# MystenLabs/dapol

Hardware: AMD Instinct MI355X
Metric: entities/sec (tree build + 64-bit range-proof gen), 2^20 leaves, 1/2/4/8 GPU (higher is better)
Workload: dtype int32 limbs (255-bit modular integers)

## Files before the change

### dapol_amd/csrc/host_range.inc

```

#include <cstdlib>
#include "policy_plan.inc"
#include "prove_plan.inc"

struct MsmTiming {
    std::vector<hipEvent_t> ev;
    std::vector<int> kind;
    size_t used = 0;
    bool enabled = false;
    size_t kernels[2] = {0, 0};
    ~MsmTiming() { for (auto e : ev) (void)hipEventDestroy(e); }
    hipError_t mark(hipStream_t st, int k = 0) {
        if (!enabled) return hipSuccess;
        if (used == ev.size()) {
            hipEvent_t e;
            hipError_t r = hipEventCreate(&e);
            if (r != hipSuccess) return r;
            ev.push_back(e);
        }
        if ((used & 1) == 0) { if (kind.size() <= used / 2) kind.push_back(k); else kind[used / 2] = k; }
        return hipEventRecord(ev[used++], st);
    }
    void count(int k, size_t n) { if (enabled) kernels[k] += n; }
    double total_ms(int k) {
// ... 159 lines not shown
        if (tm) tm->count(0, 1);
    }
}

static int32_t launch_materialise(dapol_ctx* ctx, const ProvePlan& P, const ProveLane& L, const RangeArgs& A, hipStream_t st, MsmTiming* tm) {
    const size_t cb = A.B, T = (size_t)P.tail_n;
    const unsigned g_tail = (unsigned)(cb * (size_t)(P.tail_n / 32));
    if (P.gs_mat) {
        const int LW = P.mat_LW(), cpl = P.mat_cpl(cb);
        const unsigned g_cls = nblk(cb * (size_t)LW, 64);
        const size_t slot_words = (size_t)4 * FE_NL * cb * LW;
        for (int side = 0; side < 2; side++)
            for (int c0 = 0; c0 < P.tail_n; c0 += MAT_GROUP) {
                const int nc = P.tail_n - c0 < MAT_GROUP ? P.tail_n - c0 : MAT_GROUP;
                for (int c = 0; c < nc; c += cpl) {
                    const int ny = nc - c < cpl ? nc - c : cpl;
                    hipLaunchKernelGGL(k_rp_mat_gs, dim3(g_cls, ny), dim3(64), 0, st, A, ctx->tv, side, c0 + c, 0, LW, L.gsacc + c * slot_words);
                    if (LW < A.nwin) hipLaunchKernelGGL(k_rp_mat_gs, dim3(g_cls, ny), dim3(64), 0, st, A, ctx->tv, side, c0 + c, 1, LW, L.gsacc + c * slot_words);
                }
                hipLaunchKernelGGL(k_rp_mat_gs_horner, dim3(nblk(cb * (size_t)nc, 64)), dim3(64), 0, st, A, side, c0, nc, LW, L.gsacc);
            }
        if (tm) tm->count(1, 2 * (size_t)((P.tail_n + cpl - 1) / cpl) * (LW < A.nwin ? 2 : 1));
    } else if (P.mat_split > 1) {
        RangeArgs Am = A;
        Am.nsplit = P.mat_split; Am.P0 = L.split[2];
        hipLaunchKernelGGL((k_rp_msm<MSM_MATERIALIZE, 32>), dim3(g_tail * (unsigned)P.mat_split), dim3(64), 0, st, Am, ctx->tv, -1); LAUNCH_CHECK();
        hipLaunchKernelGGL(k_rp_sum_mat, dim3(nblk(cb * 2 * T, 64)), dim3(64), 0, st, cb * 2 * T, P.mat_split, Am.P0, A.tailT);
    } else {
        hipLaunchKernelGGL((k_rp_msm<MSM_MATERIALIZE, 32>), dim3(g_tail), dim3(64), 0, st, A, ctx->tv, -1);
        if (tm) tm->count(1, 1);
    }
    LAUNCH_CHECK();
    return DAPOL_OK;
}

static int32_t queue_chunk(dapol_ctx* ctx, const ProvePlan& P, const ProveLane& L, RangeArgs A, hipStream_t st, ForkGuard& fg, uint32_t* d_err,
                           MsmTiming* tm) {
    const size_t cb = A.B;
    const int fs_shape = P.fs_shape, nf_rounds = P.nf_rounds();
    sc* const stab_buf = A.stab;
    if (!P.stab_main) A.stab = nullptr;
    const unsigned g_wave = (unsigned)cb, g_lane = nblk(cb, 64), g_dig = (unsigned)(cb * (size_t)(A.TP / 64));
    const unsigned g_gsdig = nblk(cb * (size_t)(2 * A.N), 64);
    hipLaunchKernelGGL(k_rp_nonce_key, dim3(g_lane), dim3(64), 0, st, A); LAUNCH_CHECK();
    if (P.gs) hipLaunchKernelGGL(k_rp_nonces_gs, dim3(g_gsdig), dim3(64), 0, st, A);
    else hipLaunchKernelGGL(k_rp_nonces, dim3(g_dig), dim3(64), 0, st, A);
    LAUNCH_CHECK();
    if (P.side_A) {
        HIPCHK(hipEventRecord(ctx->ev_fork, st));
        HIPCHK(hipStreamWaitEvent(ctx->side[2], ctx->ev_fork, 0));
        fg.forked(2);
        hipLaunchKernelGGL(k_rp_A, dim3(g_wave), dim3(64), 0, ctx->side[2], A, ctx->tv); LAUNCH_CHECK();
        HIPCHK(hipEventRecord(ctx->ev_join[2], ctx->side[2]));
        FAULT_AFTER_FORK("prove_A");
    } else if (P.a_lane(cb)) {
        hipLaunchKernelGGL(k_rp_A_lane, dim3(g_lane), dim3(64), 0, st, A, ctx->tv); LAUNCH_CHECK();
    } else {
        hipLaunchKernelGGL(k_rp_A, dim3(g_wave), dim3(64), 0, st, A, ctx->tv); LAUNCH_CHECK();
    }
    if (tm) HIPCHK(tm->mark(st));
    launch_main_msm(ctx, P, L, A, st, -1, tm); LAUNCH_CHECK();
    if (tm) HIPCHK(tm->mark(st));
    if (P.side_A) { HIPCHK(hipStreamWaitEvent(st, ctx->ev_join[2], 0)); fg.joined(2); }
    LAUNCH_FS(k_rp_finish1, fs_shape, cb, st, A, ctx->tv); LAUNCH_CHECK();
    hipLaunchKernelGGL(k_rp_poly, dim3(g_wave * (unsigned)A.fs_parts), dim3(64), 0, st, A); LAUNCH_CHECK();
    LAUNCH_FS(k_rp_finish2, fs_shape, cb, st, A, ctx->tv); LAUNCH_CHECK();
    hipLaunchKernelGGL(k_rp_lr, dim3(g_wave * (unsigned)A.fs_parts), dim3(64), 0, st, A); LAUNCH_CHECK();
    if (fs_shape == 2) hipLaunchKernelGGL(k_rp_finish3<2>, dim3(g_wave), dim3(64), 0, st, A);
    else hipLaunchKernelGGL(k_rp_finish3<0>, dim3(g_lane), dim3(64), 0, st, A);
    LAUNCH_CHECK();
    for (int k = 0; k < nf_rounds; k++) {
        if (P.gs) hipLaunchKernelGGL(k_rp_round_prep_gs, dim3(g_gsdig), dim3(64), 0, st, A, k);
        else hipLaunchKernelGGL(k_rp_round_prep, dim3(g_dig), dim3(64), 0, st, A, k);
        LAUNCH_CHECK();
        hipLaunchKernelGGL(k_rp_round_ip, dim3(g_wave), dim3(64), 0, st, A, k); LAUNCH_CHECK();
        if (tm) HIPCHK(tm->mark(st));
        launch_main_msm(ctx, P, L, A, st, k, tm); LAUNCH_CHECK();
        if (tm) HIPCHK(tm->mark(st));
        LAUNCH_FS(k_rp_round_finish, fs_shape, cb, st, A, ctx->tv, k); LAUNCH_CHECK();
        hipLaunchKernelGGL(k_rp_fold, dim3(fold_blocks(A, cb, k)), dim3(256), 0, st, A, k);
        LAUNCH_CHECK();
    }
    if (nf_rounds == A.lgN) {
        hipLaunchKernelGGL(k_rp_final, dim3(g_lane), dim3(64), 0, st, A, d_err); LAUNCH_CHECK();
        return DAPOL_OK;
    }
    if (P.gs_mat) hipLaunchKernelGGL(k_rp_mat_prep_gs, dim3(g_gsdig), dim3(64), 0, st, A);
    else hipLaunchKernelGGL(k_rp_mat_prep, dim3(g_dig), dim3(64), 0, st, A);
    LAUNCH_CHECK();
    if (tm) HIPCHK(tm->mark(st, 1));
    { int32_t rc = launch_materialise(ctx, P, L, A, st, tm); if (rc) return rc; }
    if (tm) HIPCHK(tm->mark(st, 1));
    const unsigned g_tail = (unsigned)(cb * (size_t)(P.tail_n / 32));
    {
        RangeArgs Ai = A;
        Ai.stab = P.stab_tail ? stab_buf : nullptr;
        if (P.tail_rpl == 4) hipLaunchKernelGGL(k_rp_tail_table4, dim3(nblk(cb * (size_t)(2 * P.tail_n / 4), 64)), dim3(64), 0, st, Ai);
        else hipLaunchKernelGGL(k_rp_tail_table, dim3(g_tail), dim3(64), 0, st, Ai);
        LAUNCH_CHECK();
    }
    RangeArgs At = A;
    At.N = P.tail_n; At.lgN = P.tail_lgn; At.TP = 2 * P.tail_n; At.wbits = TAIL_WBITS; At.nwin = TAIL_NWIN; At.nsplit = 0;
    At.a = A.tail_a; At.b = A.tail_b; At.s1 = A.tail_s1; At.s2 = A.tail_s2;
    At.stab = P.stab_tail ? stab_buf : nullptr;
    At.out_round0 = nf_rounds;
    const TableView tvt{A.tailT, 1, TAIL_WBITS, 0, 0};
    for (int k = 0; k < P.tail_lgn; k++) {
        hipLaunchKernelGGL(k_rp_round_prep, dim3(g_tail), dim3(64), 0, st, At, k); LAUNCH_CHECK();
        hipLaunchKernelGGL(k_rp_round_ip, dim3(g_wave), dim3(64), 0, st, At, k); LAUNCH_CHECK();
        if (P.tail_gs) {
            hipLaunchKernelGGL(k_rp_tail_gs, dim3(nblk(2 * cb, TAIL_GS_LISTS)), dim3(TAIL_GS_BLOCK), 0, st, At, tvt, k, L.gsacc); LAUNCH_CHECK();
            hipLaunchKernelGGL(k_rp_tail_combine, dim3(nblk(2 * cb, 64)), dim3(64), 0, st, At, L.gsacc);
        } else launch_msm_tail(st, At, tvt, k, P.tail_lpl);
        LAUNCH_CHECK();
        LAUNCH_FS(k_rp_round_finish, fs_shape, cb, st, At, ctx->tv, k); LAUNCH_CHECK();
        hipLaunchKernelGGL(k_rp_fold, dim3(fold_blocks(At, cb, k)), dim3(256), 0, st, At, k);
        LAUNCH_CHECK();
    }
    hipLaunchKernelGGL(k_rp_final, dim3(g_lane), dim3(64), 0, st, At, d_err); LAUNCH_CHECK();
    return DAPOL_OK;
}

static int32_t range_prove_device(dapol_ctx* ctx, int n, int m, size_t B, const uint64_t* d_vals, const uint32_t* d_blind,
                                  const uint32_t* d_Vc, const uint32_t* d_seed, const uint64_t* d_stream, uint64_t slot_base,
                                  const uint32_t* d_tape, uint32_t* d_out, MsmTiming* tm, size_t tape_stride = 0, uint32_t sub_k = 1,
                                  size_t out_stride = 0, PendingProve* pend = nullptr) {
    ProveShape s{};
    s.n = n; s.m = m; s.B = B;
    s.tail_length = ctx->opt.tail_length; s.small_call_max = ctx->opt.small_call_max; s.generator_stationary = ctx->opt.generator_stationary;
    s.streams = ctx->opt.streams; s.gs_tile_rows = ctx->opt.gs_tile_rows; s.gs_slices = ctx->opt.gs_slices; s.chunk_proofs = ctx->opt.chunk_proofs;
    s.wbits = ctx->tv.wbits; s.nwin = ctx->tv.nwin_c(); s.hi_split = ctx->tv.hi_split;
    s.n_cu = ctx->n_cu; s.resident_waves = ctx->resident_waves();
    s.budget_bytes = scratch_budget_bytes(ctx);
    s.timed = tm != nullptr;
    ProvePlan P = plan_range_prove(s);
    for (bool lowered = false;; lowered = true) {
        hipError_t e = ctx->scratch.ensure(P.lane_bytes() * P.nlanes);
        if (e == hipSuccess) {
            if (lowered) P.finalise(s, P.chunk, P.nlanes);
            break;
        }
        (void)hipGetLastError();
        if (e != hipErrorOutOfMemory || (P.nlanes == 1 && P.chunk <= 64)) return fail_hip(e, "scratch allocation", __FILE__, __LINE__);
        if (P.nlanes > 1) P.nlanes--;
        else P.chunk = (P.chunk + 1) / 2;
    }
    const size_t chunk = P.chunk, slots = (size_t)m * (2 * (size_t)n + 4);
    const int nlanes = P.nlanes;
    RangeArgs A{};
    A.n = n; A.m = m; A.N = P.N; A.lgN = P.lgN; A.TP = P.TP;
    A.out_words = 72 + 16 * A.lgN;
    A.seed = d_seed; A.slot_base = slot_base;
    A.wbits = s.wbits; A.nwin = s.nwin;
    A.tail_n = P.tail_n; A.use_hi = P.use_hi ? 1 : 0; A.fs_parts = P.fs_parts; A.mat_round = P.nf_rounds();
    A.stream_id = d_stream;
    A.tape_stride = (uint32_t)(tape_stride ? tape_stride : slots);
    A.tape = d_tape;
    A.sub_k = sub_k ? sub_k : 1; A.sub_slots = (uint32_t)slots;
    A.out = d_out; A.out_stride = out_stride ? out_stride : (size_t)A.out_words;
    ProveLane lanes[4];
    hipStream_t lane_stream[4] = {ctx->stream, ctx->side[0], ctx->side[1], ctx->side[2]};
    for (int ln = 0; ln < nlanes; ln++) lanes[ln] = carve_lane(P, A, (uint8_t*)ctx->scratch.p + P.lane_bytes() * ln);
    DevBuf<uint32_t> err_own;
    DevBuf<uint32_t>& err = pend ? pend->err : err_own;
    HIPCHK(err.alloc(1));
    HIPCHK(hipMemsetAsync(err.p, 0, 4, ctx->stream));
    ForkGuard fg(ctx);
    if (nlanes > 1) {
        HIPCHK(hipEventRecord(ctx->ev_fork, ctx->stream));
        for (int ln = 1; ln < nlanes; ln++) { HIPCHK(hipStreamWaitEvent(lane_stream[ln], ctx->ev_fork, 0)); fg.forked(ln - 1); }
    }
    size_t chunk_no = 0;
    for (size_t first = 0; first < B; first += chunk, chunk_no++) {
        const int ln = (int)(chunk_no % (size_t)nlanes);
        if (chunk_no == 2) FAULT_AFTER_FORK("prove_lanes");
        RangeArgs Ac = lanes[ln].A;
        Ac.B = B - first < chunk ? B - first : chunk;
        Ac.vals = d_vals + first * m;
        Ac.blind = d_blind + first * m * 8;
        Ac.Vc = d_Vc + first * m * 8;
        Ac.p0 = first;
        int32_t rc = queue_chunk(ctx, P, lanes[ln], Ac, lane_stream[ln], fg, err.p, tm);
        if (rc) return rc;
    }
    for (int ln = 1; ln < nlanes; ln++) {
        HIPCHK(hipEventRecord(ctx->ev_join[ln - 1], lane_stream[ln]));
        HIPCHK(hipStreamWaitEvent(ctx->stream, ctx->ev_join[ln - 1], 0));
        fg.joined(ln - 1);
    }
    if (pend) {
        pend->ctx = ctx;
        pend->h_err_p = ctx->h_pinned + pend->pinned_slot;
        HIPCHK(hipMemcpyAsync(pend->h_err_p, err.p, 4, hipMemcpyDeviceToHost, ctx->stream));
        pend->armed = true;
        return DAPOL_OK;
    }
    uint32_t h_err = 0;
    HIPCHK(hipMemcpyAsync(&h_err, err.p, 4, hipMemcpyDeviceToHost, ctx->stream));
    HIPCHK(hipStreamSynchronize(ctx->stream));
    if (h_err) return fail(DAPOL_ERR_INVALID_ARGUMENT, "prover drew a zero challenge (ProofError::MaliciousDealer)");
    return DAPOL_OK;
}

struct EventPair {
    hipEvent_t a = nullptr, b = nullptr;
    ~EventPair() { if (a) (void)hipEventDestroy(a); if (b) (void)hipEventDestroy(b); }
    hipError_t init() { hipError_t e = hipEventCreate(&a); return e != hipSuccess ? e : hipEventCreate(&b); }
};

int32_t dapol_range_prove_batch(dapol_ctx* ctx, int32_t n_bits, int32_t m, size_t b, const uint64_t* v, const uint8_t* r32,
                                const uint8_t nonce_seed32[32], const uint64_t* stream_id, uint64_t slot_base, const uint8_t* tape,
                                uint8_t* proofs_out) {
    if (!ctx || (b && (!v || !r32 || !proofs_out))) return fail(DAPOL_ERR_INVALID_ARGUMENT, "null argument");
    if (!tape && (!nonce_seed32 || (b && !stream_id))) return fail(DAPOL_ERR_INVALID_ARGUMENT, "seed mode needs nonce_seed32 and stream_id");
    size_t ps = dapol_range_proof_size(n_bits, m);
    if (ps == 0) return fail(DAPOL_ERR_INVALID_ARGUMENT, "n_bits must be 8/16/32/64 and m a power of two");
    if (m > ctx->max_parties) return fail(DAPOL_ERR_INVALID_ARGUMENT, "m exceeds the context's max_parties (InvalidGeneratorsLength)");
    if (b == 0) return DAPOL_OK;
    HIPCHK(hipSetDevice(ctx->device));
    hipStream_t st = ctx->stream;
    const size_t tot = b * (size_t)m, slots = (size_t)m * (2 * (size_t)n_bits + 4);
    DevBuf<uint64_t> dv, dstream;
    DevBuf<uint32_t> dr, dVc, dseed, dtape, dout;
    HIPCHK(dv.alloc(tot)); HIPCHK(dr.alloc(tot * 8)); HIPCHK(dVc.alloc(tot * 8)); HIPCHK(dseed.alloc(8));
    HIPCHK(dout.alloc(b * ps / 4));
    HIPCHK(hipMemcpyAsync(dv.p, v, tot * 8, hipMemcpyHostToDevice, st));
    HIPCHK(hipMemcpyAsync(dr.p, r32, tot * 32, hipMemcpyHostToDevice, st));
    if (tape) {
        HIPCHK(dtape.alloc(b * slots * 16));
        HIPCHK(hipMemcpyAsync(dtape.p, tape, b * slots * 64, hipMemcpyHostToDevice, st));
        HIPCHK(hipMemsetAsync(dseed.p, 0, 32, st));
    } else {
        HIPCHK(dstream.alloc(b));
        HIPCHK(hipMemcpyAsync(dstream.p, stream_id, b * 8, hipMemcpyHostToDevice, st));
        HIPCHK(hipMemcpyAsync(dseed.p, nonce_seed32, 32, hipMemcpyHostToDevice, st));
    }
    hipLaunchKernelGGL(k_rp_commit_V, dim3(nblk(tot, 256)), dim3(256), 0, st, ctx->tv, tot, dv.p, dr.p, dVc.p);
    LAUNCH_CHECK();
    EventPair ev;
    HIPCHK(ev.init());
    HIPCHK(hipEventRecord(ev.a, st));
    int32_t rc = range_prove_device(ctx, n_bits, m, b, dv.p, dr.p, dVc.p, dseed.p, dstream.p, slot_base, dtape.p, dout.p, nullptr);
    if (rc) return rc;
    HIPCHK(hipEventRecord(ev.b, st));
    HIPCHK(hipMemcpy(proofs_out, dout.p, b * ps, hipMemcpyDeviceToHost));
    { float ms = 0; if (hipEventElapsedTime(&ms, ev.a, ev.b) == hipSuccess) g_last_range_prove_ms.store((double)ms, std::memory_order_relaxed); }
    return DAPOL_OK;
}
```

### dapol_amd/csrc/kernels_range.h

```cpp
#pragma once
#include <hip/hip_runtime.h>
#include <type_traits>
#include "kernels_ctx_tree.h"
#include "ge_quad.h"

namespace dapol {

struct ProofState {
    uint64_t strobe[25];
    uint32_t pos, pos_begin;
    uint32_t err, pad_;
    sc y, z, y_inv, x, w, u, u_inv;
    sc a_bl, s_bl, t1, t2, t1_bl, t2_bl, t_x, cL, cR;
    uint32_t nkey[8];
};

struct RangeArgs {
    int n, m, N, lgN, TP;
    int wbits, nwin;
    size_t B;
    const uint64_t* vals;
    const uint32_t* blind;
    const uint32_t* Vc;
    const uint32_t* seed;
    const uint64_t* stream_id;
    uint64_t slot_base;
    const uint32_t* tape;
    uint32_t tape_stride;
    uint32_t sub_k, sub_slots;
    size_t p0;
    sc* a; sc* b; sc* s1; sc* s2;
    sc* stab;
    dig_t* dig;
    int nsplit;
    int use_hi;
    int fs_parts;
    sc* fs_part;
    ProofState* st;
    int32_t* PA; int32_t* P0; int32_t* P1;
    int mat_round;
    int tail_n;
    int32_t* tailT;
    sc* tail_a; sc* tail_b; sc* tail_s1; sc* tail_s2;
    uint32_t* out;
    size_t out_stride;
    int out_words;
    int out_round0;
};

#ifndef DAPOL_TAIL_WBITS
#define DAPOL_TAIL_WBITS 5
#endif
enum { TAIL_WBITS = DAPOL_TAIL_WBITS, TAIL_NWIN = 253 / TAIL_WBITS + 1, TAIL_ENTRIES = (1 << (TAIL_WBITS - 1)) + 1, TAIL_ROW_WORDS = TAIL_ENTRIES * 32 };
enum { MSM_PLAIN = 0, MSM_MATERIALIZE = 1, MSM_TAIL = 2 };
enum { STAB_ROUNDS = 6, STAB_N = 1 << STAB_ROUNDS };

__device__ __forceinline__ void proof_row(const RangeArgs& A, size_t b, size_t& e, uint32_t& j) {
    const size_t g = A.p0 + b;
    if (A.sub_k <= 1) { e = g; j = 0; }
    else { e = g / A.sub_k; j = (uint32_t)(g - e * A.sub_k); }
}
__device__ __forceinline__ uint32_t* proof_out(const RangeArgs& A, size_t b) {
    size_t e; uint32_t j;
    proof_row(A, b, e, j);
    return A.out + e * A.out_stride + (size_t)j * (size_t)A.out_words;
}
__device__ __forceinline__ void tape_wide(uint32_t* w16, const RangeArgs& A, size_t b, uint32_t slot) {
    size_t e; uint32_t j;
    proof_row(A, b, e, j);
    const uint32_t first = j * A.sub_slots;
    if (A.tape) {
        const uint4* p = reinterpret_cast<const uint4*>(A.tape + (e * (size_t)A.tape_stride + first + slot) * 16);
        for (int i = 0; i < 4; i++) { uint4 q = p[i]; w16[4 * i] = q.x; w16[4 * i + 1] = q.y; w16[4 * i + 2] = q.z; w16[4 * i + 3] = q.w; }
    } else {
        uint32_t key[8];
        for (int i = 0; i < 8; i++) key[i] = A.st[b].nkey[i];
        seed_wide(w16, key, 2u, A.stream_id[e], A.slot_base + first + slot);
    }
}
__global__ __launch_bounds__(64) void k_rp_nonce_key(RangeArgs A) {
    size_t b = (size_t)blockIdx.x * 64 + threadIdx.x;
    if (b >= A.B || A.tape) return;
    uint32_t key[8], w[16];
    for (int i = 0; i < 8; i++) key[i] = A.seed[i];
    size_t e; uint32_t sj;
    proof_row(A, b, e, sj);
    seed_wide(w, key, 6u, A.stream_id[e], A.slot_base + (uint64_t)sj * A.sub_slots);
    for (int i = 0; i < 8; i++) key[i] = w[i];
    seed_wide(w, key, 7u, (uint64_t)A.n, (uint64_t)A.m);
    for (int i = 0; i < 8; i++) key[i] = w[i];
    for (int j0 = 0; j0 < A.m; j0 += 31) {
        const int n_ent = 1 + ((A.m - j0 < 31) ? A.m - j0 : 31);
        const int n_blk = (n_ent + 1) / 2;
        uint32_t cv[8], blk[16], o[16];
        blake3_iv(cv);
        for (int i = 0; i < n_blk; i++) {
            for (int h = 0; h < 2; h++) {
                const int e = 2 * i + h;
                if (e == 0) { for (int k = 0; k < 8; k++) blk[k] = key[k]; }
                else if (e < n_ent) ld8(blk + 8 * h, A.Vc + (b * A.m + j0 + e - 1) * 8);
                else { for (int k = 0; k < 8; k++) blk[8 + k] = 0; }
            }
            const bool last = i == n_blk - 1;
            blake3_compress(o, cv, blk, 0, (last && (n_ent & 1)) ? 32u : 64u, (i == 0 ? B3_CHUNK_START : 0u) | (last ? (B3_CHUNK_END | B3_ROOT) : 0u));
            for (int k = 0; k < 8; k++) cv[k] = o[k];
        }
        for (int k = 0; k < 8; k++) key[k] = cv[k];
    }
    for (int i = 0; i < 8; i++) A.st[b].nkey[i] = key[i];
}
__device__ __forceinline__ void tape_scalar(sc& r, const RangeArgs& A, size_t b, uint32_t slot) {
    uint32_t w[16];
    tape_wide(w, A, b, slot);
    sc_from_wide(r, w);
}
__device__ __forceinline__ void ld_sc(sc& r, const sc* p) {
    const uint4* q = reinterpret_cast<const uint4*>(p);
    uint4 a = q[0], b = q[1];
    r.v[0] = a.x; r.v[1] = a.y; r.v[2] = a.z; r.v[3] = a.w; r.v[4] = b.x; r.v[5] = b.y; r.v[6] = b.z; r.v[7] = b.w;
}
__device__ __forceinline__ void st_sc(sc* p, const sc& r) {
    uint4* q = reinterpret_cast<uint4*>(p);
    q[0] = make_uint4(r.v[0], r.v[1], r.v[2], r.v[3]);
    q[1] = make_uint4(r.v[4], r.v[5], r.v[6], r.v[7]);
}
__device__ __forceinline__ void write_digits_plain(const RangeArgs& A, size_t b, int pos, const uint32_t* c) {
    dig_t* d = A.dig + (size_t)b * A.nwin * A.TP + pos;
    const int TP = A.TP;
    sc_recode_w(A.wbits, A.nwin, c, [&](int i, int digit) { d[(size_t)i * TP] = (dig_t)digit; });
}
__device__ __forceinline__ void write_digits(const RangeArgs& A, size_t b, int pos, const sc& s_mont) {
    uint32_t c[8];
    sc_from_mont(c, s_mont);
    write_digits_plain(A, b, pos, c);
}
__device__ __forceinline__ void zero_digits(const RangeArgs& A, size_t b, int pos) {
    dig_t* d = A.dig + (size_t)b * A.nwin * A.TP + pos;
    for (int i = 0; i < A.nwin; i++) d[(size_t)i * A.TP] = 0;
}

__device__ __forceinline__ void coeff_times(sc& p, const RangeArgs& A, size_t b, int round, int j, bool isH, const sc& v) {
    if (A.stab) {
        const sc* T = A.stab + ((b * 2 + (size_t)(round & 1)) * 2 + (isH ? 1 : 0)) * STAB_N + (round ? (j >> (A.lgN - round)) : 0);
        sc t;
        ld_sc(t, T);
        if (isH) {
            sc yi, q;
            ld_sc(yi, A.s2 + b * A.N + j);
            sc_montmul(q, v, yi);
            sc_montmul(p, q, t);
        } else sc_montmul(p, v, t);
    } else {
        sc sv;
        ld_sc(sv, (isH ? A.s2 : A.s1) + b * A.N + j);
        sc_montmul(p, v, sv);
    }
}
__device__ __forceinline__ void coeff_plain(sc& s, const RangeArgs& A, size_t b, int round, int j, bool isH) {
    if (A.stab) {
        const sc* T = A.stab + ((b * 2 + (size_t)(round & 1)) * 2 + (isH ? 1 : 0)) * STAB_N + (round ? (j >> (A.lgN - round)) : 0);
        sc t;
        ld_sc(t, T);
        if (isH) {
            sc yi;
            ld_sc(yi, A.s2 + b * A.N + j);
            sc_montmul(s, yi, t);
        } else s = t;
    } else ld_sc(s, (isH ? A.s2 : A.s1) + b * A.N + j);
}
__device__ __forceinline__ void stab_init(const RangeArgs& A, size_t b) {
    if (!A.stab) return;
    sc one_p, one_m;
    sc_zero(one_p); one_p.v[0] = 1;
    sc_one_mont(one_m);
    st_sc(A.stab + (b * 2 * 2 + 0) * STAB_N, one_p);
    st_sc(A.stab + (b * 2 * 2 + 1) * STAB_N, one_m);
}

__device__ __forceinline__ int term_generator(int round, int N, int lgN, int side, int q, bool& isH) {
    if (round < 0) {
        isH = side != 0;
        return q;
    }
    int lgh = lgN - 1 - round;
    int half = 1 << lgh, Nh = N >> 1;
    isH = q >= Nh;
// ... 944 lines not shown
```

### dapol_amd/csrc/kernels_range_gs.h

```cpp
#pragma once
#include "kernels_range.h"

namespace dapol {

__device__ __forceinline__ void write_digits_gs(const RangeArgs& A, size_t p, int sp, const uint32_t* c) {
    const size_t L = A.B * (size_t)A.nwin;
    int32_t* out = reinterpret_cast<int32_t*>(A.dig) + ((((size_t)(sp >> 2)) * L + p) << 2) + (sp & 3);
    const size_t wstride = A.B * (size_t)4;
    const int W = A.wbits, NW = A.nwin, half = 1 << (W - 1);
    const uint32_t mask = (1u << W) - 1;
    uint32_t x[8];
#pragma unroll
    for (int i = 0; i < 8; i++) x[i] = c[i];
    int carry = 0;
#pragma nounroll
    for (int w = 0; w < NW; w++) {
        const int b = (int)(x[0] & mask) + carry;
        carry = (b >= half && w != NW - 1) ? 1 : 0;
        out[(size_t)w * wstride] = b - (carry << W);
#pragma unroll
        for (int i = 0; i < 7; i++) x[i] = (x[i] >> W) | (x[i + 1] << (32 - W));
        x[7] >>= W;
    }
}

#define GS_BLOCKS(A, vb) for (size_t vb = blockIdx.x, nb_ = ((size_t)(A).B * (size_t)(2 * (A).N) + 63) / 64; vb < nb_; vb += gridDim.x)
__device__ __forceinline__ bool gs_thread(const RangeArgs& A, size_t vblock, size_t& p, int& sp) {
    const size_t t = vblock * 64 + threadIdx.x;
    const size_t quad = t >> 2, sp4 = quad / A.B;
    p = quad - sp4 * A.B;
    sp = (int)(4 * sp4) + (int)(t & 3);
    return sp4 < (size_t)(2 * A.N) / 4;
}

__global__ __launch_bounds__(64) void k_rp_nonces_gs(RangeArgs A) {
    GS_BLOCKS(A, vb) {
        size_t p;
        int sp;
        if (!gs_thread(A, vb, p, sp)) continue;
        const int side = sp >= A.N ? 1 : 0, q = sp - side * A.N;
        const int j = q / A.n, ii = q - j * A.n;
        const uint32_t slot = (uint32_t)(j * (2 * A.n + 2) + 2 + ii + (side ? A.n : 0));
        sc s;
        tape_scalar(s, A, p, slot);
        st_sc((side ? A.s2 : A.s1) + p * A.N + q, s);
        uint32_t c[8];
        sc_from_mont(c, s);
        write_digits_gs(A, p, sp, c);
    }
}

__global__ __launch_bounds__(64) void k_rp_round_prep_gs(RangeArgs A, int round) {
    GS_BLOCKS(A, vb) {
        size_t p;
        int sp;
        if (!gs_thread(A, vb, p, sp)) continue;
        const int side = sp >= A.N ? 1 : 0, q = sp - side * A.N;
        const int lgh = A.lgN - 1 - round, half = 1 << lgh;
        bool isH;
        const int j = term_generator(round, A.N, A.lgN, side, q, isH);
        const int off = j & (half - 1);
        const bool upper = (j >> lgh) & 1;
        const int vi = upper ? off : off + half;
        sc v, pr;
        ld_sc(v, (isH ? A.b : A.a) + p * A.N + vi);
        coeff_times(pr, A, p, round, j, isH, v);
        write_digits_gs(A, p, sp, pr.v);
    }
}

#ifndef DAPOL_GS_OCC
#define DAPOL_GS_OCC 4
#endif
__global__ __launch_bounds__(64, DAPOL_GS_OCC) void k_rp_msm_gs(RangeArgs A, TableView tbl, int round, int side, int q0, int nq, int first, int32_t* __restrict__ accs, int slice_rows) {
    const size_t L = A.B * (size_t)A.nwin, Ltot = L * gridDim.y;
    const size_t lane = (size_t)blockIdx.x * 64 + threadIdx.x;
    if (lane >= L) return;
    q0 += (int)blockIdx.y * slice_rows;
    ge_p3 acc;
    int32_t* ap = accs + (size_t)blockIdx.y * L + lane;
    if (first) ge_identity(acc);
    else {
#pragma unroll
        for (int i = 0; i < FE_NL; i++) {
            acc.X.v[i] = ap[(size_t)i * Ltot]; acc.Y.v[i] = ap[(size_t)(FE_NL + i) * Ltot];
            acc.Z.v[i] = ap[(size_t)(2 * FE_NL + i) * Ltot]; acc.T.v[i] = ap[(size_t)(3 * FE_NL + i) * Ltot];
        }
    }
    const dapol_v4i* dg = reinterpret_cast<const dapol_v4i*>(A.dig) + ((size_t)(side * A.N + q0) >> 2) * L + lane;
    dapol_v4i d4 = dg[0], dn = d4;
#pragma nounroll
    for (int i = 0; i < nq; i++) {
        if ((i & 3) == 0 && i + 4 < nq) dn = dg[(size_t)((i >> 2) + 1) * L];
        const int d = d4.x;
        d4.x = d4.y; d4.y = d4.z; d4.z = d4.w;
        if ((i & 3) == 3) d4 = dn;
        bool isH;
        const int j = term_generator(round, A.N, A.lgN, side, q0 + i, isH);
        tbl_madd(acc, tbl, gen_row(tbl, A.n, j, isH), d);
    }
#pragma unroll
    for (int i = 0; i < FE_NL; i++) {
        ap[(size_t)i * Ltot] = acc.X.v[i]; ap[(size_t)(FE_NL + i) * Ltot] = acc.Y.v[i];
        ap[(size_t)(2 * FE_NL + i) * Ltot] = acc.Z.v[i]; ap[(size_t)(3 * FE_NL + i) * Ltot] = acc.T.v[i];
    }
}

__global__ __launch_bounds__(64, DAPOL_GS_OCC) void k_rp_msm_gs_hi(RangeArgs A, TableView tbl, int round, int side, int q0, int nq, int first, int32_t* __restrict__ accs,
                                                                  int slice_rows, int LW) {
    const size_t L = A.B * (size_t)LW, Ltot = L * gridDim.y, Ld = A.B * (size_t)A.nwin;
    const size_t lane = (size_t)blockIdx.x * 64 + threadIdx.x;
    if (lane >= L) return;
    q0 += (int)blockIdx.y * slice_rows;
    const int w = (int)(lane / A.B);
    const bool has_hi = w + LW < A.nwin;
    ge_p3 acc;
    int32_t* ap = accs + (size_t)blockIdx.y * L + lane;
    if (first) ge_identity(acc);
    else {
#pragma unroll
        for (int i = 0; i < FE_NL; i++) {
            acc.X.v[i] = ap[(size_t)i * Ltot]; acc.Y.v[i] = ap[(size_t)(FE_NL + i) * Ltot];
            acc.Z.v[i] = ap[(size_t)(2 * FE_NL + i) * Ltot]; acc.T.v[i] = ap[(size_t)(3 * FE_NL + i) * Ltot];
        }
    }
    const dapol_v4i* dg = reinterpret_cast<const dapol_v4i*>(A.dig) + ((size_t)(side * A.N + q0) >> 2) * Ld + lane;
    const dapol_v4i* dh = dg + (has_hi ? (size_t)LW * A.B : 0);
    dapol_v4i d4 = dg[0], h4 = dh[0], dn = d4, hn = h4;
#pragma nounroll
    for (int i2 = 0; i2 < 2 * nq; i2++) {
        const int i = i2 >> 1, hi = i2 & 1;
        if (!hi && (i & 3) == 0 && i + 4 < nq) { dn = dg[(size_t)((i >> 2) + 1) * Ld]; hn = dh[(size_t)((i >> 2) + 1) * Ld]; }
        int d;
        if (!hi) { d = d4.x; d4.x = d4.y; d4.y = d4.z; d4.z = d4.w; }
        else {
            d = h4.x;
            h4.x = h4.y; h4.y = h4.z; h4.z = h4.w;
            if ((i & 3) == 3) { d4 = dn; h4 = hn; }
            if (!has_hi) continue;
        }
        bool isH;
        const int j = term_generator(round, A.N, A.lgN, side, q0 + i, isH);
        const int row = gen_row(tbl, A.n, j, isH);
        tbl_madd(acc, tbl, hi ? tbl.row_hi(row) : row, d);
    }
#pragma unroll
    for (int i = 0; i < FE_NL; i++) {
        ap[(size_t)i * Ltot] = acc.X.v[i]; ap[(size_t)(FE_NL + i) * Ltot] = acc.Y.v[i];
        ap[(size_t)(2 * FE_NL + i) * Ltot] = acc.Z.v[i]; ap[(size_t)(3 * FE_NL + i) * Ltot] = acc.T.v[i];
    }
}

__global__ __launch_bounds__(64) void k_rp_gs_sum_slices(RangeArgs A, int32_t* __restrict__ accs, size_t side_words, int nslice, int LW) {
    const size_t L = A.B * (size_t)LW, Ltot = L * (size_t)nslice;
    const size_t t = (size_t)blockIdx.x * 64 + threadIdx.x;
    if (t >= 2 * L) return;
    const int side = t >= L ? 1 : 0;
    int32_t* ap = accs + (size_t)side * side_words + (t - (size_t)side * L);
    auto load = [&](ge_p3& r, int s) {
        const int32_t* q = ap + (size_t)s * L;
        for (int i = 0; i < FE_NL; i++) {
            r.X.v[i] = q[(size_t)i * Ltot]; r.Y.v[i] = q[(size_t)(FE_NL + i) * Ltot];
            r.Z.v[i] = q[(size_t)(2 * FE_NL + i) * Ltot]; r.T.v[i] = q[(size_t)(3 * FE_NL + i) * Ltot];
        }
    };
    ge_p3 acc, o, r;
    load(acc, 0);
#pragma nounroll
    for (int s = 1; s < nslice; s++) {
        load(o, s);
        ge_add(r, acc, o);
        acc = r;
    }
    for (int i = 0; i < FE_NL; i++) {
        ap[(size_t)i * Ltot] = acc.X.v[i]; ap[(size_t)(FE_NL + i) * Ltot] = acc.Y.v[i];
        ap[(size_t)(2 * FE_NL + i) * Ltot] = acc.Z.v[i]; ap[(size_t)(3 * FE_NL + i) * Ltot] = acc.T.v[i];
    }
}

__global__ __launch_bounds__(64) void k_rp_gs_combine(RangeArgs A, const int32_t* __restrict__ accs, size_t side_words, int nslice, int LW) {
    const size_t Ltot = A.B * (size_t)LW * (size_t)nslice;
    const size_t t = (size_t)blockIdx.x * 64 + threadIdx.x;
    if (t >= 2 * A.B) return;
    const int side = t >= A.B ? 1 : 0;
    const size_t p = t - (size_t)side * A.B;
    accs += (size_t)side * side_words;
    auto load = [&](ge_p3& r, int w) {
        const int32_t* ap = accs + (size_t)w * A.B + p;
        for (int i = 0; i < FE_NL; i++) {
            r.X.v[i] = ap[(size_t)i * Ltot]; r.Y.v[i] = ap[(size_t)(FE_NL + i) * Ltot];
            r.Z.v[i] = ap[(size_t)(2 * FE_NL + i) * Ltot]; r.T.v[i] = ap[(size_t)(3 * FE_NL + i) * Ltot];
        }
    };
    ge_p3 acc, t2, r;
    load(acc, LW - 1);
#pragma nounroll
    for (int w = LW - 2; w >= 0; w--) {
#pragma nounroll
        for (int d = 0; d < A.wbits; d++) ge_dbl(acc, acc, d == A.wbits - 1);
        load(t2, w);
        ge_add(r, acc, t2);
        acc = r;
    }
    st_p3((side ? A.P1 : A.P0) + p * 40, acc);
}

enum { MAT_GROUP = 16 };
enum { GS_ACC_SLOTS = 32, GS_MAX_SLICES = 16, GS_FULL_LANES = 3072 * 64 };
static_assert(GS_ACC_SLOTS >= MAT_GROUP && GS_ACC_SLOTS >= 2 * GS_MAX_SLICES, "accumulator slots");

__global__ __launch_bounds__(64) void k_rp_mat_prep_gs(RangeArgs A) {
    GS_BLOCKS(A, vb) {
        size_t p;
        int sp;
        if (!gs_thread(A, vb, p, sp)) continue;
        const int side = sp >= A.N ? 1 : 0, rem = sp - side * A.N;
        const int per = A.N / A.tail_n, cls = rem / per, k = rem - cls * per;
        sc s;
        coeff_plain(s, A, p, A.mat_round, cls + k * A.tail_n, side != 0);
        write_digits_gs(A, p, sp, s.v);
    }
}

__global__ __launch_bounds__(64, DAPOL_GS_OCC) void k_rp_mat_gs(RangeArgs A, TableView tbl, int side, int cls, int hi, int LW, int32_t* __restrict__ accs) {
    const size_t LM = A.B * (size_t)LW, L = A.B * (size_t)A.nwin;
    const size_t lane = (size_t)blockIdx.x * 64 + threadIdx.x;
    if (lane >= LM) return;
    cls += (int)blockIdx.y;
    accs += (size_t)blockIdx.y * 4 * FE_NL * LM;
    const int w = (int)(lane / A.B);
    const size_t p = lane - (size_t)w * A.B;
    const int wd = w + (hi ? LW : 0);
    if (wd >= A.nwin) return;
    ge_p3 acc;
    int32_t* ap = accs + lane;
    if (!hi) ge_identity(acc);
    else {
#pragma unroll
        for (int i = 0; i < FE_NL; i++) {
            acc.X.v[i] = ap[(size_t)i * LM]; acc.Y.v[i] = ap[(size_t)(FE_NL + i) * LM];
            acc.Z.v[i] = ap[(size_t)(2 * FE_NL + i) * LM]; acc.T.v[i] = ap[(size_t)(3 * FE_NL + i) * LM];
        }
    }
    const int per = A.N / A.tail_n;
    const dapol_v4i* dg = reinterpret_cast<const dapol_v4i*>(A.dig) + ((size_t)(side * A.N + cls * per) >> 2) * L + (size_t)wd * A.B + p;
    dapol_v4i d4 = dg[0], dn = d4;
#pragma nounroll
    for (int k = 0; k < per; k++) {
        if ((k & 3) == 0 && k + 4 < per) dn = dg[(size_t)((k >> 2) + 1) * L];
        const int d = d4.x;
        d4.x = d4.y; d4.y = d4.z; d4.z = d4.w;
        if ((k & 3) == 3) d4 = dn;
        const int row = gen_row(tbl, A.n, cls + k * A.tail_n, side != 0);
        tbl_madd(acc, tbl, hi ? tbl.row_hi(row) : row, d);
    }
#pragma unroll
    for (int i = 0; i < FE_NL; i++) {
        ap[(size_t)i * LM] = acc.X.v[i]; ap[(size_t)(FE_NL + i) * LM] = acc.Y.v[i];
        ap[(size_t)(2 * FE_NL + i) * LM] = acc.Z.v[i]; ap[(size_t)(3 * FE_NL + i) * LM] = acc.T.v[i];
    }
}

__global__ __launch_bounds__(64) void k_rp_mat_gs_horner(RangeArgs A, int side, int cls0, int ncls, int LW, const int32_t* __restrict__ accs) {
    const size_t LM = A.B * (size_t)LW;
    const size_t t = (size_t)blockIdx.x * 64 + threadIdx.x;
    if (t >= (size_t)ncls * A.B) return;
    const int c = (int)(t / A.B);
    const size_t p = t - (size_t)c * A.B;
    const int32_t* slot = accs + (size_t)c * 4 * FE_NL * LM;
    auto load = [&](ge_p3& r, int w) {
        const int32_t* ap = slot + (size_t)w * A.B + p;
        for (int i = 0; i < FE_NL; i++) {
            r.X.v[i] = ap[(size_t)i * LM]; r.Y.v[i] = ap[(size_t)(FE_NL + i) * LM];
            r.Z.v[i] = ap[(size_t)(2 * FE_NL + i) * LM]; r.T.v[i] = ap[(size_t)(3 * FE_NL + i) * LM];
        }
    };
    ge_p3 acc, q, r;
    load(acc, LW - 1);
#pragma nounroll
    for (int w = LW - 2; w >= 0; w--) {
#pragma nounroll
        for (int d = 0; d < A.wbits; d++) ge_dbl(acc, acc, d == A.wbits - 1);
        load(q, w);
        ge_add(r, acc, q);
        acc = r;
    }
    const int T = A.tail_n;
    st_p3(A.tailT + (p * (size_t)(2 * T) + (size_t)(side * T + cls0 + c)) * TAIL_ROW_WORDS, acc);
}

enum { TAIL_GS_BLOCK = 256, TAIL_GS_LISTS = TAIL_GS_BLOCK / TAIL_NWIN, TAIL_REC_WORDS = 4 * FE_NL };
static_assert(TAIL_GS_LISTS >= 1, "a list's windows fit a block");
__global__ __launch_bounds__(TAIL_GS_BLOCK, DAPOL_GS_OCC) void k_rp_tail_gs(RangeArgs A, TableView tbl, int round, int32_t* __restrict__ recs) {
    const int li = (int)threadIdx.x / TAIL_NWIN, w = (int)threadIdx.x - li * TAIL_NWIN;
    const size_t list = (size_t)blockIdx.x * TAIL_GS_LISTS + li;
    if (li >= TAIL_GS_LISTS || list >= 2 * A.B) return;
    const size_t p = list >> 1;
    const int side = (int)(list & 1);
    tbl.base += p * (size_t)(2 * A.N) * tbl.row_words();
    const dig_t* dw = A.dig + (p * A.nwin + (size_t)w) * (size_t)A.TP + 32 * side;
    ge_p3 acc;
    ge_identity(acc);
    dapol_v4i d4 = *reinterpret_cast<const dapol_v4i*>(dw), dn = d4;
#pragma nounroll
    for (int q = 0; q < A.N; q++) {
        if ((q & 3) == 0 && q + 4 < A.N) dn = *reinterpret_cast<const dapol_v4i*>(dw + 64 * ((q + 4) >> 5) + ((q + 4) & 31));
        const int d = d4.x;
        d4.x = d4.y; d4.y = d4.z; d4.z = d4.w;
        if ((q & 3) == 3) d4 = dn;
        bool isH;
        const int j = term_generator(round, A.N, A.lgN, side, q, isH);
        tbl_madd(acc, tbl, j + (isH ? A.N : 0), d);
    }
    st_p3(recs + (list * TAIL_NWIN + (size_t)w) * TAIL_REC_WORDS, acc);
}

__global__ __launch_bounds__(64) void k_rp_tail_combine(RangeArgs A, const int32_t* __restrict__ recs) {
    const size_t list = (size_t)blockIdx.x * 64 + threadIdx.x;
    if (list >= 2 * A.B) return;
    const int32_t* rp = recs + list * TAIL_NWIN * TAIL_REC_WORDS;
    ge_p3 acc, t2, r;
    ld_p3(acc, rp + (size_t)(A.nwin - 1) * TAIL_REC_WORDS);
#pragma nounroll
    for (int w = A.nwin - 2; w >= 0; w--) {
#pragma nounroll
        for (int d = 0; d < A.wbits; d++) ge_dbl(acc, acc, d == A.wbits - 1);
        ld_p3(t2, rp + (size_t)w * TAIL_REC_WORDS);
        ge_add(r, acc, t2);
        acc = r;
    }
    st_p3(((list & 1) ? A.P1 : A.P0) + (list >> 1) * 40, acc);
}

}
```

### dapol_amd/csrc/sc.h

```cpp
#pragma once
#include "consts.h"

namespace dapol {

struct sc {
    uint32_t v[8];
};

DAPOL_HD void sc_zero(sc& r) {
    for (int i = 0; i < 8; i++) r.v[i] = 0;
}
DAPOL_HD void sc_one_mont(sc& r) {
    for (int i = 0; i < 8; i++) r.v[i] = SC_R1[i];
}
DAPOL_HD bool sc_is_zero(const sc& a) {
    uint32_t o = 0;
    for (int i = 0; i < 8; i++) o |= a.v[i];
    return o == 0;
}

DAPOL_HD uint32_t sc_addc(uint32_t a, uint32_t b, uint32_t cin, uint32_t& cout) {
#if defined(__clang__) && !defined(DAPOL_SC_NO_BUILTIN_CARRY)
    return __builtin_addc(a, b, cin, &cout);
#else
// ... 126 lines not shown
    sc_montmul(lo, lo, k);
    for (int i = 0; i < 8; i++) k.v[i] = SC_R3[i];
    sc_montmul(hi, hi, k);
    sc_add(r, lo, hi);
}
DAPOL_HD void sc_from_mont(uint32_t* out, const sc& a) {
    sc one, r;
    sc_zero(one);
    one.v[0] = 1;
    sc_montmul(r, a, one);
    for (int i = 0; i < 8; i++) out[i] = r.v[i];
}
DAPOL_HD void sc_from_u64_mont(sc& r, uint64_t x) {
    uint32_t w[8] = {(uint32_t)x, (uint32_t)(x >> 32), 0, 0, 0, 0, 0, 0};
    sc_to_mont(r, w);
}

DAPOL_HD_NOINLINE void sc_invert_mont(sc& r, const sc& a) {
    sc acc;
    sc_one_mont(acc);
    for (int i = 252; i >= 0; i--) {
        sc_montsq(acc, acc);
        if ((SC_LM2[i >> 5] >> (i & 31)) & 1) sc_montmul(acc, acc, a);
    }
    r = acc;
}
DAPOL_HD void sc_divsteps30_var(int32_t& eta, uint32_t f, uint32_t g, int32_t* t) {
    uint32_t u = 1, v = 0, q = 0, r = 1;
    int i = 30;
    for (;;) {
        const int zeros = __builtin_ctz(g | (0xffffffffu << i));
        g >>= zeros; u <<= zeros; v <<= zeros;
        eta -= zeros; i -= zeros;
        if (i == 0) break;
        if (eta < 0) {
            eta = -eta;
            uint32_t tmp = f; f = g; g = 0u - tmp;
            tmp = u; u = q; q = 0u - tmp;
            tmp = v; v = r; r = 0u - tmp;
        }
        g += f; q += u; r += v;
    }
    t[0] = (int32_t)u; t[1] = (int32_t)v; t[2] = (int32_t)q; t[3] = (int32_t)r;
}
DAPOL_HD_NOINLINE void sc_invert_vartime_mont(sc& out, const sc& a) {
    const int32_t M30 = (int32_t)0x3fffffff;
    int32_t d[9], e[9], f[9], g[9];
    for (int i = 0; i < 9; i++) { d[i] = 0; e[i] = 0; f[i] = SC_L30[i]; }
    e[0] = 1;
    for (int i = 0; i < 9; i++) {
        const int o = 30 * i, w = o >> 5, sh = o & 31;
        uint64_t x = (uint64_t)a.v[w] | (w + 1 < 8 ? (uint64_t)a.v[w + 1] << 32 : 0ull);
        g[i] = (int32_t)((uint32_t)(x >> sh) & (uint32_t)M30);
    }
    int32_t eta = -1;
    for (int it = 0; it < 40; it++) {
        int32_t t[4];
        sc_divsteps30_var(eta, (uint32_t)f[0] | ((uint32_t)f[1] << 30), (uint32_t)g[0] | ((uint32_t)g[1] << 30), t);
        const int64_t u = t[0], v = t[1], q = t[2], r = t[3];
        {
            const int32_t sd = d[8] >> 31, se = e[8] >> 31;
            int32_t md = (t[0] & sd) + (t[1] & se), me = (t[2] & sd) + (t[3] & se);
            int64_t cd = u * d[0] + v * e[0], ce = q * d[0] + r * e[0];
            md -= (int32_t)((SC_LINV30 * (uint32_t)cd + (uint32_t)md) & (uint32_t)M30);
            me -= (int32_t)((SC_LINV30 * (uint32_t)ce + (uint32_t)me) & (uint32_t)M30);
            cd += (int64_t)SC_L30[0] * md; ce += (int64_t)SC_L30[0] * me;
            cd >>= 30; ce >>= 30;
            for (int i = 1; i < 9; i++) {
                cd += u * d[i] + v * e[i] + (int64_t)SC_L30[i] * md;
                ce += q * d[i] + r * e[i] + (int64_t)SC_L30[i] * me;
                d[i - 1] = (int32_t)cd & M30; e[i - 1] = (int32_t)ce & M30;
                cd >>= 30; ce >>= 30;
            }
            d[8] = (int32_t)cd; e[8] = (int32_t)ce;
        }
        {
            int64_t cf = u * f[0] + v * g[0], cg = q * f[0] + r * g[0];
            cf >>= 30; cg >>= 30;
            for (int i = 1; i < 9; i++) {
                cf += u * f[i] + v * g[i];
                cg += q * f[i] + r * g[i];
                f[i - 1] = (int32_t)cf & M30; g[i - 1] = (int32_t)cg & M30;
                cf >>= 30; cg >>= 30;
            }
            f[8] = (int32_t)cf; g[8] = (int32_t)cg;
        }
        int32_t nz = 0;
        for (int i = 0; i < 9; i++) nz |= g[i];
        if (nz == 0) break;
    }
    uint32_t w[9];
    {
        uint64_t acc = 0;
        int bits = 0, j = 0;
        for (int i = 0; i < 9; i++) {
            acc |= (uint64_t)(i < 8 ? (uint32_t)(d[i] & M30) : (uint32_t)d[8]) << bits;
            bits += i < 8 ? 30 : 32;
            while (bits >= 32) { w[j++] = (uint32_t)acc; acc >>= 32; bits -= 32; }
        }
        w[8] = (uint32_t)(((int32_t)((uint32_t)acc << 16)) >> 16);
    }
    if (f[8] < 0) {
        uint32_t c = 1;
        for (int i = 0; i < 9; i++) w[i] = sc_addc(~w[i], 0u, c, c);
    }
    for (int k = 0; k < 4 && (w[8] >> 31); k++) {
        uint32_t c = 0;
        for (int i = 0; i < 9; i++) w[i] = sc_addc(w[i], i < 8 ? SC_L[i] : 0u, c, c);
    }
    for (int k = 0; k < 4; k++) {
        uint32_t t9[9], bw = 0;
        for (int i = 0; i < 9; i++) t9[i] = sc_subb(w[i], i < 8 ? SC_L[i] : 0u, bw, bw);
        if (t9[8] >> 31) break;
        for (int i = 0; i < 9; i++) w[i] = t9[i];
    }
    sc x, k3;
    for (int i = 0; i < 8; i++) { x.v[i] = w[i]; k3.v[i] = SC_R3[i]; }
    sc_montmul(out, x, k3);
}

DAPOL_HD void sc_pow_mont(sc& r, const sc& a, uint32_t e) {
    sc acc, base = a;
    sc_one_mont(acc);
    while (e) {
        if (e & 1) sc_montmul(acc, acc, base);
        sc_montsq(base, base);
        e >>= 1;
    }
    r = acc;
}

DAPOL_HD void sc_recode_s8(int16_t* d, const uint32_t* x) {
    int carry = 0;
    for (int i = 0; i < 32; i++) {
        int b = (int)((x[i >> 2] >> (8 * (i & 3))) & 0xff) + carry;
        carry = (b > 127 && i < 31) ? 1 : 0;
        d[i] = (int16_t)(b - (carry << 8));
    }
}

template <typename F>
DAPOL_HD void sc_recode_w(int W, int NW, const uint32_t* x, F out) {
    int carry = 0;
    for (int i = 0; i < NW; i++) {
        int o = i * W, wd = o >> 5, sh = o & 31;
        uint32_t lo = wd < 8 ? x[wd] >> sh : 0u;
        uint32_t hi = (sh && wd + 1 < 8) ? (x[wd + 1] << (32 - sh)) : 0u;
        int b = (int)((lo | hi) & ((1u << W) - 1)) + carry;
        carry = (b >= (1 << (W - 1)) && i < NW - 1) ? 1 : 0;
        out(i, b - (carry << W));
    }
}

}
```

Before: 58220.

## Store biased scalars instead of per-window signed digits and extract windows in MSM

The digit producers now add a constant bias to each scalar and write its eight raw 32-bit words, instead of the signed-digit recoding with one int per window. The MSM and matrix kernels extract each window on the fly with an alignbit and subtract a half-window offset. This is the standard bias trick for carry-free signed digits. It cuts digit-buffer writes from nwin words to 8 words per scalar and removes the serial recoding loop. In exchange each MSM lane may issue a second quad load when its window straddles a word boundary, and does a few more ALU ops per digit.

```diff
diff --git a/dapol_amd/csrc/host_range.inc b/dapol_amd/csrc/host_range.inc
--- a/dapol_amd/csrc/host_range.inc
+++ b/dapol_amd/csrc/host_range.inc
@@ -335,6 +335,7 @@
     A.out_words = 72 + 16 * A.lgN;
     A.seed = d_seed; A.slot_base = slot_base;
     A.wbits = s.wbits; A.nwin = s.nwin;
+    sc_window_bias(A.wbits, A.nwin, A.gs_bias);
     A.tail_n = P.tail_n; A.use_hi = P.use_hi ? 1 : 0; A.fs_parts = P.fs_parts; A.mat_round = P.nf_rounds();
     A.stream_id = d_stream;
     A.tape_stride = (uint32_t)(tape_stride ? tape_stride : slots);
diff --git a/dapol_amd/csrc/kernels_range.h b/dapol_amd/csrc/kernels_range.h
--- a/dapol_amd/csrc/kernels_range.h
+++ b/dapol_amd/csrc/kernels_range.h
@@ -32,6 +32,7 @@
     sc* a; sc* b; sc* s1; sc* s2;
     sc* stab;
     dig_t* dig;
+    uint32_t gs_bias[8];
     int nsplit;
     int use_hi;
     int fs_parts;
diff --git a/dapol_amd/csrc/kernels_range_gs.h b/dapol_amd/csrc/kernels_range_gs.h
--- a/dapol_amd/csrc/kernels_range_gs.h
+++ b/dapol_amd/csrc/kernels_range_gs.h
@@ -3,25 +3,33 @@
 
 namespace dapol {
 
-__device__ __forceinline__ void write_digits_gs(const RangeArgs& A, size_t p, int sp, const uint32_t* c) {
-    const size_t L = A.B * (size_t)A.nwin;
-    int32_t* out = reinterpret_cast<int32_t*>(A.dig) + ((((size_t)(sp >> 2)) * L + p) << 2) + (sp & 3);
-    const size_t wstride = A.B * (size_t)4;
-    const int W = A.wbits, NW = A.nwin, half = 1 << (W - 1);
-    const uint32_t mask = (1u << W) - 1;
+__device__ __forceinline__ void write_biased_gs(const RangeArgs& A, size_t p, int sp, const uint32_t* c) {
     uint32_t x[8];
-#pragma unroll
-    for (int i = 0; i < 8; i++) x[i] = c[i];
-    int carry = 0;
-#pragma nounroll
-    for (int w = 0; w < NW; w++) {
-        const int b = (int)(x[0] & mask) + carry;
-        carry = (b >= half && w != NW - 1) ? 1 : 0;
-        out[(size_t)w * wstride] = b - (carry << W);
-#pragma unroll
-        for (int i = 0; i < 7; i++) x[i] = (x[i] >> W) | (x[i + 1] << (32 - W));
-        x[7] >>= W;
-    }
+    sc_add_bias(x, c, A.gs_bias);
+    uint32_t* out = reinterpret_cast<uint32_t*>(A.dig) + ((((size_t)(sp >> 2)) * 8 * A.B + p) << 2) + (sp & 3);
+    const size_t kstride = A.B * (size_t)4;
+#pragma unroll
+    for (int k = 0; k < 8; k++) out[(size_t)k * kstride] = x[k];
+}
+
+typedef sc_window GsWindow;
+__device__ __forceinline__ GsWindow gs_window(const RangeArgs& A, int w) { return sc_window_of(A.wbits, A.nwin, w); }
+__device__ __forceinline__ int gs_lane_window(size_t lane, size_t cb, size_t& p) {
+    const size_t w = ((lane | cb) >> 32) == 0 ? (size_t)((uint32_t)lane / (uint32_t)cb) : lane / cb;
+    p = lane - w * cb;
+    return (int)w;
+}
+__device__ __forceinline__ void gs_load_quad(const dapol_v4i* q, size_t cb, const GsWindow& g, dapol_v4i& lo, dapol_v4i& hi) {
+    lo = q[0];
+    if (g.two) hi = q[cb];
+}
+__device__ __forceinline__ dapol_v4i gs_quad_digits(const GsWindow& g, const dapol_v4i& lo, const dapol_v4i& hi) {
+    dapol_v4i d;
+    d.x = sc_biased_window(g, (uint32_t)lo.x, (uint32_t)hi.x);
+    d.y = sc_biased_window(g, (uint32_t)lo.y, (uint32_t)hi.y);
+    d.z = sc_biased_window(g, (uint32_t)lo.z, (uint32_t)hi.z);
+    d.w = sc_biased_window(g, (uint32_t)lo.w, (uint32_t)hi.w);
+    return d;
 }
 
 #define GS_BLOCKS(A, vb) for (size_t vb = blockIdx.x, nb_ = ((size_t)(A).B * (size_t)(2 * (A).N) + 63) / 64; vb < nb_; vb += gridDim.x)
@@ -46,7 +54,7 @@
         st_sc((side ? A.s2 : A.s1) + p * A.N + q, s);
         uint32_t c[8];
         sc_from_mont(c, s);
-        write_digits_gs(A, p, sp, c);
+        write_biased_gs(A, p, sp, c);
     }
 }
 
@@ -65,7 +73,7 @@
         sc v, pr;
         ld_sc(v, (isH ? A.b : A.a) + p * A.N + vi);
         coeff_times(pr, A, p, round, j, isH, v);
-        write_digits_gs(A, p, sp, pr.v);
+        write_biased_gs(A, p, sp, pr.v);
     }
 }
 
@@ -87,17 +95,23 @@
             acc.Z.v[i] = ap[(size_t)(2 * FE_NL + i) * Ltot]; acc.T.v[i] = ap[(size_t)(3 * FE_NL + i) * Ltot];
         }
     }
-    const dapol_v4i* dg = reinterpret_cast<const dapol_v4i*>(A.dig) + ((size_t)(side * A.N + q0) >> 2) * L + lane;
-    dapol_v4i d4 = dg[0], dn = d4;
+    size_t p;
+    const GsWindow g = gs_window(A, gs_lane_window(lane, A.B, p));
+    const size_t qs = 8 * A.B;
+    const dapol_v4i* dg = reinterpret_cast<const dapol_v4i*>(A.dig) + (((size_t)(side * A.N + q0) >> 2) * 8 + (size_t)g.k0) * A.B + p;
+    dapol_v4i d4, hi = {0, 0, 0, 0};
+    gs_load_quad(dg, A.B, g, d4, hi);
+    d4 = gs_quad_digits(g, d4, hi);
 #pragma nounroll
     for (int i = 0; i < nq; i++) {
-        if ((i & 3) == 0 && i + 4 < nq) dn = dg[(size_t)((i >> 2) + 1) * L];
         const int d = d4.x;
         d4.x = d4.y; d4.y = d4.z; d4.z = d4.w;
-        if ((i & 3) == 3) d4 = dn;
+        const bool more = (i & 3) == 3 && i + 1 < nq;
+        if (more) gs_load_quad(dg + (size_t)((i >> 2) + 1) * qs, A.B, g, d4, hi);
         bool isH;
         const int j = term_generator(round, A.N, A.lgN, side, q0 + i, isH);
         tbl_madd(acc, tbl, gen_row(tbl, A.n, j, isH), d);
+        if (more) d4 = gs_quad_digits(g, d4, hi);
     }
 #pragma unroll
     for (int i = 0; i < FE_NL; i++) {
@@ -108,11 +122,12 @@
 
 __global__ __launch_bounds__(64, DAPOL_GS_OCC) void k_rp_msm_gs_hi(RangeArgs A, TableView tbl, int round, int side, int q0, int nq, int first, int32_t* __restrict__ accs,
                                                                   int slice_rows, int LW) {
-    const size_t L = A.B * (size_t)LW, Ltot = L * gridDim.y, Ld = A.B * (size_t)A.nwin;
+    const size_t L = A.B * (size_t)LW, Ltot = L * gridDim.y;
     const size_t lane = (size_t)blockIdx.x * 64 + threadIdx.x;
     if (lane >= L) return;
     q0 += (int)blockIdx.y * slice_rows;
-    const int w = (int)(lane / A.B);
+    size_t p;
+    const int w = gs_lane_window(lane, A.B, p);
     const bool has_hi = w + LW < A.nwin;
     ge_p3 acc;
     int32_t* ap = accs + (size_t)blockIdx.y * L + lane;
@@ -124,25 +139,33 @@
             acc.Z.v[i] = ap[(size_t)(2 * FE_NL + i) * Ltot]; acc.T.v[i] = ap[(size_t)(3 * FE_NL + i) * Ltot];
         }
     }
-    const dapol_v4i* dg = reinterpret_cast<const dapol_v4i*>(A.dig) + ((size_t)(side * A.N + q0) >> 2) * Ld + lane;
-    const dapol_v4i* dh = dg + (has_hi ? (size_t)LW * A.B : 0);
-    dapol_v4i d4 = dg[0], h4 = dh[0], dn = d4, hn = h4;
+    const GsWindow g = gs_window(A, w), gh = gs_window(A, has_hi ? w + LW : w);
+    const size_t qs = 8 * A.B;
+    const dapol_v4i* dq = reinterpret_cast<const dapol_v4i*>(A.dig) + ((size_t)(side * A.N + q0) >> 2) * qs + p;
+    const dapol_v4i* dg = dq + (size_t)g.k0 * A.B;
+    const dapol_v4i* dh = dq + (size_t)gh.k0 * A.B;
+    dapol_v4i d4, h4, hi = {0, 0, 0, 0}, hhi = {0, 0, 0, 0};
+    gs_load_quad(dg, A.B, g, d4, hi);
+    gs_load_quad(dh, A.B, gh, h4, hhi);
+    d4 = gs_quad_digits(g, d4, hi); h4 = gs_quad_digits(gh, h4, hhi);
 #pragma nounroll
     for (int i2 = 0; i2 < 2 * nq; i2++) {
-        const int i = i2 >> 1, hi = i2 & 1;
-        if (!hi && (i & 3) == 0 && i + 4 < nq) { dn = dg[(size_t)((i >> 2) + 1) * Ld]; hn = dh[(size_t)((i >> 2) + 1) * Ld]; }
+        const int i = i2 >> 1, hi2 = i2 & 1;
         int d;
-        if (!hi) { d = d4.x; d4.x = d4.y; d4.y = d4.z; d4.z = d4.w; }
-        else {
-            d = h4.x;
-            h4.x = h4.y; h4.y = h4.z; h4.z = h4.w;
-            if ((i & 3) == 3) { d4 = dn; h4 = hn; }
-            if (!has_hi) continue;
-        }
-        bool isH;
-        const int j = term_generator(round, A.N, A.lgN, side, q0 + i, isH);
-        const int row = gen_row(tbl, A.n, j, isH);
-        tbl_madd(acc, tbl, hi ? tbl.row_hi(row) : row, d);
+        if (!hi2) { d = d4.x; d4.x = d4.y; d4.y = d4.z; d4.z = d4.w; }
+        else { d = h4.x; h4.x = h4.y; h4.y = h4.z; h4.z = h4.w; }
+        const bool more = hi2 && (i & 3) == 3 && i + 1 < nq;
+        if (more) {
+            gs_load_quad(dg + (size_t)((i >> 2) + 1) * qs, A.B, g, d4, hi);
+            gs_load_quad(dh + (size_t)((i >> 2) + 1) * qs, A.B, gh, h4, hhi);
+        }
+        if (!hi2 || has_hi) {
+            bool isH;
+            const int j = term_generator(round, A.N, A.lgN, side, q0 + i, isH);
+            const int row = gen_row(tbl, A.n, j, isH);
+            tbl_madd(acc, tbl, hi2 ? tbl.row_hi(row) : row, d);
+        }
+        if (more) { d4 = gs_quad_digits(g, d4, hi); h4 = gs_quad_digits(gh, h4, hhi); }
     }
 #pragma unroll
     for (int i = 0; i < FE_NL; i++) {
@@ -218,18 +241,18 @@
         const int per = A.N / A.tail_n, cls = rem / per, k = rem - cls * per;
         sc s;
         coeff_plain(s, A, p, A.mat_round, cls + k * A.tail_n, side != 0);
-        write_digits_gs(A, p, sp, s.v);
+        write_biased_gs(A, p, sp, s.v);
     }
 }
 
 __global__ __launch_bounds__(64, DAPOL_GS_OCC) void k_rp_mat_gs(RangeArgs A, TableView tbl, int side, int cls, int hi, int LW, int32_t* __restrict__ accs) {
-    const size_t LM = A.B * (size_t)LW, L = A.B * (size_t)A.nwin;
+    const size_t LM = A.B * (size_t)LW;
     const size_t lane = (size_t)blockIdx.x * 64 + threadIdx.x;
     if (lane >= LM) return;
     cls += (int)blockIdx.y;
     accs += (size_t)blockIdx.y * 4 * FE_NL * LM;
-    const int w = (int)(lane / A.B);
-    const size_t p = lane - (size_t)w * A.B;
+    size_t p;
+    const int w = gs_lane_window(lane, A.B, p);
     const int wd = w + (hi ? LW : 0);
     if (wd >= A.nwin) return;
     ge_p3 acc;
@@ -243,16 +266,21 @@
         }
     }
     const int per = A.N / A.tail_n;
-    const dapol_v4i* dg = reinterpret_cast<const dapol_v4i*>(A.dig) + ((size_t)(side * A.N + cls * per) >> 2) * L + (size_t)wd * A.B + p;
-    dapol_v4i d4 = dg[0], dn = d4;
+    const GsWindow g = gs_window(A, wd);
+    const size_t qs = 8 * A.B;
+    const dapol_v4i* dg = reinterpret_cast<const dapol_v4i*>(A.dig) + (((size_t)(side * A.N + cls * per) >> 2) * 8 + (size_t)g.k0) * A.B + p;
+    dapol_v4i d4, whi = {0, 0, 0, 0};
+    gs_load_quad(dg, A.B, g, d4, whi);
+    d4 = gs_quad_digits(g, d4, whi);
 #pragma nounroll
     for (int k = 0; k < per; k++) {
-        if ((k & 3) == 0 && k + 4 < per) dn = dg[(size_t)((k >> 2) + 1) * L];
         const int d = d4.x;
         d4.x = d4.y; d4.y = d4.z; d4.z = d4.w;
-        if ((k & 3) == 3) d4 = dn;
+        const bool more = (k & 3) == 3 && k + 1 < per;
+        if (more) gs_load_quad(dg + (size_t)((k >> 2) + 1) * qs, A.B, g, d4, whi);
         const int row = gen_row(tbl, A.n, cls + k * A.tail_n, side != 0);
         tbl_madd(acc, tbl, hi ? tbl.row_hi(row) : row, d);
+        if (more) d4 = gs_quad_digits(g, d4, whi);
     }
 #pragma unroll
     for (int i = 0; i < FE_NL; i++) {
diff --git a/dapol_amd/csrc/sc.h b/dapol_amd/csrc/sc.h
--- a/dapol_amd/csrc/sc.h
+++ b/dapol_amd/csrc/sc.h
@@ -302,4 +302,38 @@
     }
 }
 
-}
+DAPOL_HD void sc_window_bias(int W, int NW, uint32_t* K) {
+    for (int k = 0; k < 8; k++) K[k] = 0;
+    for (int w = 0; w < NW - 1; w++) {
+        const int b = W * w + W - 1;
+        if (b < 256) K[b >> 5] |= 1u << (b & 31);
+    }
+}
+DAPOL_HD void sc_add_bias(uint32_t* r, const uint32_t* x, const uint32_t* K) {
+    uint32_t c = 0;
+    for (int k = 0; k < 8; k++) r[k] = sc_addc(x[k], K[k], c, c);
+}
+struct sc_window {
+    int k0, sh, half;
+    uint32_t mask;
+    bool two;
+};
+DAPOL_HD sc_window sc_window_of(int W, int NW, int w) {
+    sc_window g;
+    const int bit = W * w;
+    g.k0 = bit >> 5; g.sh = bit & 31;
+    g.mask = (1u << W) - 1;
+    g.half = w < NW - 1 ? 1 << (W - 1) : 0;
+    g.two = g.sh + W > 32 && g.k0 + 1 < 8;
+    return g;
+}
+DAPOL_HD int sc_biased_window(const sc_window& g, uint32_t lo, uint32_t hi) {
+#if defined(__HIP_DEVICE_COMPILE__)
+    const uint32_t v = __builtin_amdgcn_alignbit(hi, lo, (uint32_t)g.sh);
+#else
+    const uint32_t v = (uint32_t)((((uint64_t)hi << 32) | lo) >> g.sh);
+#endif
+    return (int)(v & g.mask) - g.half;
+}
+
+}
```

Result: no change. 58600 (median of 6 runs) (+0.6%).
